# qimingfan10/Prov-gigapath-replication

Measured on AMD Instinct MI355X. Metric: slide-encoder tiles/sec at 1/2/4/8 GPUs (12L768d LongNet); attn MFMA util %, higher is better.
Workload: dtype bf16; 1 GPU; C3: gigapath_slide_enc12l768d forward, one 70000-tile slide per GPU, all_layer_embed=True; slides_per_gpu=1, parallelism=replica x1

## Files before the change

### include/gigapath_hip.h

```cpp
#ifndef GIGAPATH_HIP_H
#define GIGAPATH_HIP_H

#include <stddef.h>
#include <stdint.h>

#ifdef __cplusplus
extern "C" {
#endif

#define GP_ABI_VERSION 10
#define GP_EARG (-1)
#define GP_MAX_BRANCHES 8
#define GP_MAX_DESTS 8

#define GP_FMT_BF16 0
#define GP_FMT_F16 1
#define GP_FMT_F16_VBF16 2

int gp_abi_version(void);

const char* gp_last_error_string(void);

int gp_coords_to_pos(const void* coords, int coords_is_f64, int64_t n_tiles, int grid,
                     double tile_size, int64_t* pos, int32_t* err_count, void* stream);

// ... 63 lines not shown
int gp_branch_merge_ln_window(const uint16_t* const* o_in, const float* const* lse_in,
                              const int32_t* seg_len, const int32_t* ratios, int nbranch, int64_t B,
                              int64_t L, int64_t tok_lo, int64_t n_tok, int H, int D, const float* ln_w,
                              const float* ln_b, float eps, uint16_t* out, int fmt, void* stream);

int64_t gp_varlen_plan_bytes(int nslide, int nbranch);
int gp_varlen_plan(const int64_t* L, int nslide, int H, int D, const int32_t* seg_len,
                   const int32_t* ratios, int nbranch, const uint16_t* qkv, int64_t qkv_row_stride,
                   uint16_t* const* o_out, float* const* lse_out, void* plan_host, int64_t plan_bytes,
                   int64_t* o_elems, int64_t* lse_elems);
int gp_dilated_attn_fwd_varlen(const void* plan_host, const void* plan_dev, int q_log2_prescaled,
                               int fmt, void* stream);
int gp_branch_merge_ln_varlen(const void* plan_host, const void* plan_dev, const float* ln_w,
                              const float* ln_b, float eps, uint16_t* out, int fmt, void* stream);

int gp_residual_layernorm(float* x, const uint16_t* y, const float* bias, const float* ln_w,
                          const float* ln_b, float eps, uint16_t* ln_out, int64_t rows, int cols,
                          int fmt, void* stream);

int gp_residual2_layernorm(float* x, const uint16_t* y1, const float* b1, const uint16_t* y2, const float* b2,
                           const float* ln_w, const float* ln_b, float eps, uint16_t* ln_out, int64_t rows,
                           int cols, int fmt, void* stream);

int gp_gelu_layernorm(const uint16_t* h, const float* ln_w, const float* ln_b, float eps,
                      uint16_t* out, int64_t rows, int cols, int fmt, void* stream);

int64_t gp_gemm_workspace_bytes(int64_t M, int64_t N, int64_t K);

int gp_linear(const uint16_t* A, int64_t lda, const uint16_t* W, int64_t ldw, const float* bias,
              uint16_t* C, int64_t ldc, int64_t M, int64_t N, int64_t K, void* ws, int64_t ws_bytes,
// ... 43 lines not shown
```

### prov-gigapath-replication_amd/gigapath/_hip.py

```python
from __future__ import annotations

import ctypes
import os
from typing import Optional, Sequence

import torch

_HERE = os.path.dirname(os.path.abspath(__file__))
LIB_PATH = os.path.join(_HERE, "_lib", "libgigapath_hip.so")
ABI_VERSION = 10
MAX_BRANCHES = 8
MAX_DESTS = 8

c_i32, c_i64, c_f32, c_f64, c_vp = ctypes.c_int32, ctypes.c_int64, ctypes.c_float, ctypes.c_double, ctypes.c_void_p


class GpRowDest(ctypes.Structure):
    _fields_ = [("tok_lo", c_i64), ("tok_hi", c_i64), ("dst", c_vp)]


class GpAttnBranch(ctypes.Structure):
    _fields_ = [("seg_len", c_i32), ("ratio", c_i32), ("k", c_vp), ("v", c_vp), ("kv_row_stride", c_i64),
                ("kv_tok_base", c_i64), ("kv_sparse_cols", c_i32), ("o", c_vp), ("lse", c_vp),
                ("key_part", c_i32), ("key_parts", c_i32)]

# ... 7 lines not shown
    "gp_dilated_attn_fwd": [c_vp, c_vp, c_vp, c_i64, c_i64, c_i64, c_i32, c_i32, c_vp, c_vp, c_i32, c_vp, c_vp,
                            c_f32, c_i32, c_i32, c_vp],
    "gp_dilated_attn_fwd_ex": [c_vp, c_i64, c_i64, c_i64, c_i64, c_i32, c_i32, c_i64, c_i64, c_vp, c_i32, c_f32,
                               c_i32, c_i32, c_vp],
    "gp_attn_launch_params": [c_vp, c_i32],
    "gp_dilated_sparsify": [c_vp, c_i64, c_i64, c_i64, c_i64, c_i64, c_i64, c_i32, c_i32, c_vp, c_vp, c_i32, c_vp,
                            c_vp, c_vp],
    "gp_dilated_sparsify_dests": [c_vp, c_i64, c_i64, c_i64, c_i64, c_i64, c_i64, c_i32, c_i32, c_vp, c_vp, c_i32,
                                  c_vp, c_vp, c_vp],
    "gp_branch_merge_ln_window": [c_vp, c_vp, c_vp, c_vp, c_i32, c_i64, c_i64, c_i64, c_i64, c_i32, c_i32, c_vp, c_vp,
                                  c_f32, c_vp, c_i32, c_vp],
    "gp_seg_attn_fwd": [c_vp, c_vp, c_vp, c_i64, c_i64, c_i32, c_i32, c_f32, c_vp, c_vp, c_vp],
    "gp_seg_attn_fwd_f16": [c_vp, c_vp, c_vp, c_i64, c_i64, c_i32, c_i32, c_f32, c_vp, c_vp, c_vp],
    "gp_branch_merge_ln": [c_vp, c_vp, c_vp, c_vp, c_i32, c_i64, c_i64, c_i32, c_i32, c_vp, c_vp, c_f32, c_vp, c_i32,
                           c_vp],
    "gp_residual_layernorm": [c_vp, c_vp, c_vp, c_vp, c_vp, c_f32, c_vp, c_i64, c_i32, c_i32, c_vp],
    "gp_residual2_layernorm": [c_vp, c_vp, c_vp, c_vp, c_vp, c_vp, c_vp, c_f32, c_vp, c_i64, c_i32, c_i32, c_vp],
    "gp_gelu_layernorm": [c_vp, c_vp, c_vp, c_f32, c_vp, c_i64, c_i32, c_i32, c_vp],
    "gp_layernorm_f32": [c_vp, c_i64, c_vp, c_vp, c_f32, c_vp, c_i64, c_i32, c_vp],
    "gp_mean_tokens": [c_vp, c_i64, c_i64, c_i32, c_i64, c_vp, c_vp],
    "gp_varlen_plan_bytes": [c_i32, c_i32],
    "gp_varlen_plan": [c_vp, c_i32, c_i32, c_i32, c_vp, c_vp, c_i32, c_vp, c_i64, c_vp, c_vp, c_vp, c_i64, c_vp, c_vp],
    "gp_dilated_attn_fwd_varlen": [c_vp, c_vp, c_i32, c_i32, c_vp],
    "gp_branch_merge_ln_varlen": [c_vp, c_vp, c_vp, c_vp, c_f32, c_vp, c_i32, c_vp],
    "gp_gemm_workspace_bytes": [c_i64, c_i64, c_i64],
    "gp_linear": [c_vp, c_i64, c_vp, c_i64, c_vp, c_vp, c_i64, c_i64, c_i64, c_i64, c_vp, c_i64, c_i32, c_vp],
    "gp_ffn_fc1_gelu": [c_vp, c_i64, c_vp, c_i64, c_vp, c_vp, c_i64, c_vp, c_i64, c_i64, c_i64, c_i32, c_vp],
    "gp_ffn_fc2_ln": [c_vp, c_i64, c_vp, c_i64, c_vp, c_vp, c_vp, c_f32, c_vp, c_i64, c_i64, c_i64, c_i64, c_vp, c_i64,
                      c_i32, c_vp],
    "gp_linear_resid": [c_vp, c_i64, c_vp, c_i64, c_vp, c_vp, c_i64, c_vp, c_vp, c_vp, c_i64, c_vp, c_f32, c_vp, c_i64,
                        c_i64, c_i64, c_vp, c_i64, c_i32, c_vp],
    "gp_linear_ln": [c_vp, c_i64, c_vp, c_i64, c_vp, c_i32, c_vp, c_vp, c_f32, c_vp, c_vp, c_vp, c_i64, c_i64, c_i64,
                     c_i64, c_vp, c_i64, c_i32, c_vp],
    "gp_ffn_fc1_gelu_ln": [c_vp, c_i64, c_vp, c_i64, c_vp, c_i32, c_vp, c_vp, c_f32, c_vp, c_vp, c_vp, c_i64, c_vp,
                           c_i64, c_i64, c_i64, c_i32, c_vp],
    "gp_ffn_fc2_ln_resid": [c_vp, c_i64, c_vp, c_i64, c_vp, c_vp, c_vp, c_f32, c_vp, c_i64, c_vp, c_vp, c_vp, c_i64,
                            c_vp, c_f32, c_vp, c_i64, c_i64, c_i64, c_vp, c_i64, c_i32, c_vp],
}
_RESTYPES = {"gp_last_error_string": ctypes.c_char_p, "gp_varlen_plan_bytes": c_i64, "gp_gemm_workspace_bytes": c_i64}

_lib = None


class HipLibraryError(RuntimeError):
    pass


def load_library(path: Optional[str] = None) -> ctypes.CDLL:
    global _lib
    if _lib is not None and path is None:
        return _lib
    p = path or LIB_PATH
    if not os.path.exists(p):
        raise HipLibraryError(
# ... 209 lines not shown
        (lib.gp_seg_attn_fwd, "gp_seg_attn_fwd")
    _check(fn(_ptr(q), _ptr(k), _ptr(v), nb, sl, H, D, float(softmax_scale), _ptr(o), _ptr(lse), _stream()), name)


def branch_merge_ln(outs, lses, segs, ratios, B, L, H, D, ln_w, ln_b, eps, out):
    lib = load_library()
    fmt = fmt_of(out.dtype)
    _dev(out, name="out")
    for o in outs:
        _dev(o, out.dtype, "o")
    _check(lib.gp_branch_merge_ln(_ptr_array(outs), _ptr_array(lses), _i32_array(segs), _i32_array(ratios),
                                  len(segs), B, L, H, D, _ptr(ln_w), _ptr(ln_b), eps, _ptr(out), fmt, _stream()),
           "gp_branch_merge_ln")


def residual_layernorm(x, y, bias, ln_w, ln_b, eps, ln_out, rows, cols):
    lib = load_library()
    fmt = fmt_of(y.dtype)
    _dev(x, torch.float32, "x"); _dev(y, name="y")
    if ln_out is not None:
        _dev(ln_out, y.dtype, "ln_out")
    _check(lib.gp_residual_layernorm(_ptr(x), _ptr(y), _ptr(bias), _ptr(ln_w), _ptr(ln_b), eps, _ptr(ln_out),
                                     rows, cols, fmt, _stream()), "gp_residual_layernorm")


def residual2_layernorm(x, y1, b1, y2, b2, ln_w, ln_b, eps, ln_out, rows, cols):
    lib = load_library()
    fmt = fmt_of(y1.dtype)
    _dev(x, torch.float32, "x"); _dev(y1, name="y1")
    if y2 is not None:
# ... 252 lines not shown
```

### prov-gigapath-replication_amd/gigapath/runtime.py

```python
from __future__ import annotations

import functools
import math
import os
import threading
from collections import OrderedDict
from dataclasses import dataclass, field
from typing import Dict, List, Optional, Sequence, Tuple

import numpy as np
import torch

from . import _hip

_TUNED = os.path.join(os.path.dirname(os.path.abspath(__file__)), "tuned", "tunableop_results.csv")
_tuned_loaded = False


def use_tuned_gemms(dev=None):
    global _tuned_loaded
    path = os.environ.get("GIGAPATH_TUNED_GEMMS_FILE", _TUNED)
    if _tuned_loaded or os.environ.get("GIGAPATH_NO_TUNED_GEMMS") == "1" or not os.path.exists(path):
        return
    if dev is None or torch.device(dev).type != "cuda":
# ... 325 lines not shown
    with TIMER.span("gemm_out"):
        _hip.linear_resid(ws.a, pa.w_o, pa.b_o, ws.x, ws.shift[0], pl.ln2_w, ws.y, ws.xstats, ws.gemm_ws,
                          eps_next=pl.ln2_eps if mp else None, s_out=ws.shift[1] if mp else None)
    with TIMER.span("gemm_fc1"):
        _hip.ffn_fc1_gelu_ln(ws.y, pl.w1, ws.xstats, E // 256, pl.c1, pl.d1, pl.ln2_eps, ws.shift[0], ws.shift[1],
                             ws.f, ws.fstats, merged=mp)
    with TIMER.span("gemm_fc2"):
        last = nxt is None
        _hip.ffn_fc2_ln_resid(ws.f, pl.w2g, ws.fstats, pl.c2, pl.d2, pl.fln_eps, ws.x, ws.shift[1],
                              None if last else nxt.ln1_w, ws.y, ws.xstats, ws.gemm_ws,
                              eps_next=None if (last or not mp) else nxt.ln1_eps,
                              s_out=None if (last or not mp) else ws.shift[0])


def ffn_forward(pl: "PackedLayer", a: torch.Tensor, f: torch.Tensor, y: torch.Tensor, fstats, gemm_ws,
                M: int, F: int) -> Optional[torch.Tensor]:
    if pl.ffn_fused and fstats is not None:
        with TIMER.span("gemm_fc1"):
            _hip.ffn_fc1_gelu(a, pl.w1, pl.b1_f32, f, fstats)
        with TIMER.span("gemm_fc2"):
            _hip.ffn_fc2_ln(f, pl.w2g, fstats, pl.c2, pl.d2, pl.fln_eps, y, gemm_ws)
        return None
    with TIMER.span("gemm_fc1"), blaslt_serialized():
        torch.addmm(pl.b1, a, pl.w1.t(), out=f)
    with TIMER.span("gelu_ln"):
        _hip.gelu_layernorm(f, pl.fln_w, pl.fln_b, pl.fln_eps, f, M, F)
    with TIMER.span("gemm_fc2"), blaslt_serialized():
        torch.mm(f, pl.w2.t(), out=y)
    return pl.b2


def ffn_buffers(dev, M: int, E: int, F: int):
    if not (ffn_fusable(E, F) or resid_fusable(E, F)):
        return None, gemm_workspace(dev, M, E, F)
    stats = torch.empty((F // 256 + 1) * M * 2, dtype=torch.float32, device=dev)
    return stats, gemm_workspace(dev, M, E, F)


def gemm_workspace(dev, M: int, E: int, F: int) -> torch.Tensor:
    nb = 0
    if torch.device(dev).type == "cuda":
        shapes = [(E, F)] + ([(3 * E, E), (E, E)] if OWN_GEMMS else [])
# ... 32 lines not shown
            raise RuntimeError("varlen packing needs the pre-scaled q of D = 48")
        with TIMER.span("attn"):
            _hip.dilated_attn_fwd_varlen(scratch.plan, True, v_bf16=v_bf16)
        with TIMER.span("merge"):
            _hip.branch_merge_ln_varlen(scratch.plan, pa.ln_w if inner_ln else None, pa.ln_b if inner_ln else None,
                                        pa.ln_eps, out)
        return
    with TIMER.span("attn"):
        _hip.dilated_attn_fwd(qkv, qkv[:, E:], qkv[:, 2 * E:], 3 * E, B, L, H, D, pa.segs, pa.ratios,
                              scratch.outs, scratch.lses, 0.0, pa.prescaled, v_bf16=v_bf16)
    with TIMER.span("merge"):
        _hip.branch_merge_ln(scratch.outs, scratch.lses, pa.segs, pa.ratios, B, L, H, D,
                             pa.ln_w if inner_ln else None, pa.ln_b if inner_ln else None, pa.ln_eps, out)


class Workspace:
    def __init__(self, dev, B: int, L: int, E: int, F: int, H: int, segs, ratios, act: torch.dtype = torch.bfloat16):
        M = B * L
        self.key = (str(dev), B, L, E, F, H, tuple(segs), tuple(ratios), act)
        self.x = torch.empty(M, E, dtype=torch.float32, device=dev)
        self.a = torch.empty(M, E, dtype=act, device=dev)
        self.qkv = torch.empty(M, 3 * E, dtype=act, device=dev)
        self.y = torch.empty(M, E, dtype=act, device=dev)
        self.y2 = torch.empty(M, E, dtype=act, device=dev)
        self.f = torch.empty(M, F, dtype=act, device=dev)
        self.fstats, self.gemm_ws = ffn_buffers(dev, M, E, F)
        self.xstats, self.shift = resid_buffers(dev, M, E)
        self.attn = AttentionScratch(dev, B, L, H, E // H, segs, ratios, act)


class PackedWorkspace(Workspace):
# ... 4 lines not shown
        T = sum(self.Ls)
        M = T
        self.key = (str(dev), tuple(self.Ls), E, F, H, tuple(segs), tuple(ratios), act)
        self.x = torch.empty(M, E, dtype=torch.float32, device=dev)
        self.a = torch.empty(M, E, dtype=act, device=dev)
        self.qkv = torch.empty(M, 3 * E, dtype=act, device=dev)
        self.y = torch.empty(M, E, dtype=act, device=dev)
        self.y2 = torch.empty(M, E, dtype=act, device=dev)
        self.f = torch.empty(M, F, dtype=act, device=dev)
        self.fstats, self.gemm_ws = ffn_buffers(dev, M, E, F)
        self.xstats, self.shift = resid_buffers(dev, M, E)
        self.attn = VarlenScratch(dev, self.Ls, H, E // H, segs, ratios, self.qkv)
        self.tok_off = self.attn.plan.tok_off
        self.cls_idx = torch.tensor(self.tok_off[:-1], dtype=torch.int64, device=dev)


class EncoderEngine:

    def __init__(self):
        self._sig = None
        self.layers: List[PackedLayer] = []
        self._packs: Dict[torch.dtype, tuple] = {}
        self._ws: "OrderedDict[int, Workspace]" = OrderedDict()
        self._pws: "OrderedDict[int, PackedWorkspace]" = OrderedDict()
        self.ws: Optional[Workspace] = None
        self.pws: Optional[PackedWorkspace] = None

    def pack(self, encoder, dev, act: Optional[torch.dtype] = None):
        use_tuned_gemms(dev)
        act = act or act_dtype()
# ... 40 lines not shown
        return self.pws

    def stream_workspace(self, stream, packed: bool = False):
        table = self._pws if packed else self._ws
        return table.get(int(stream.cuda_stream)) if stream is not None else None

    def detach_workspace(self, ws) -> None:
        for table in (self._ws, self._pws):
            for k in [k for k, v in table.items() if v is ws]:
                table.pop(k)
        if self.ws is ws:
            self.ws = None
        if self.pws is ws:
            self.pws = None

    def run_layers(self, ws: Workspace, B: int, L: int, layer_hook=None, shift_ready: bool = False):
        M = B * L
        E = ws.x.shape[1]
        F = ws.f.shape[1]
        nl = len(self.layers)
        if self.layers and all(pl.resid_fused for pl in self.layers) and ws.fstats is not None:
            if not shift_ready:
                torch.mean(ws.x, 1, out=ws.shift[0])
            for li, pl in enumerate(self.layers):
                pa = pl.attn
                with TIMER.span("gemm_qkv"):
                    if li == 0:
                        linear(ws.a, pa.w_qkv, pa.b_qkv, pa.b_qkv_f32, ws.qkv, ws.gemm_ws, v_bf16=pa.v_bf16)
                    else:
                        fused_qkv(pl, ws, ws.qkv)
                dilated_attention_core(pa, ws.qkv, B, L, ws.attn, ws.a, v_bf16=pa.v_bf16)
                fused_post_attention(pl, self.layers[li + 1] if li + 1 < nl else None, ws)
                if layer_hook is not None:
                    layer_hook(li + 1)
            return
        for li, pl in enumerate(self.layers):
            pa = pl.attn
            with TIMER.span("gemm_qkv"):
                linear(ws.a, pa.w_qkv, pa.b_qkv, pa.b_qkv_f32, ws.qkv, ws.gemm_ws, v_bf16=pa.v_bf16)
            dilated_attention_core(pa, ws.qkv, B, L, ws.attn, ws.a, v_bf16=pa.v_bf16)
            with TIMER.span("gemm_out"):
                linear(ws.a, pa.w_o, None, None, ws.y, ws.gemm_ws)
            nxt = self.layers[li + 1] if li + 1 < nl else None
            residual_pair(pl, nxt, ws, M, E, F)
            if layer_hook is not None:
                layer_hook(li + 1)


RESID2 = os.environ.get("GIGAPATH_RESID2", "1") != "0"


def residual_pair(pl: "PackedLayer", nxt: Optional["PackedLayer"], ws, M: int, E: int, F: int):
    pa = pl.attn
    ln1 = (nxt.ln1_w, nxt.ln1_b, nxt.ln1_eps) if nxt else (None, None, 1e-5)
    if RESID2:
        with TIMER.span("resid_ln"):
            _hip.residual2_layernorm(ws.x, ws.y, pa.b_o, None, None, pl.ln2_w, pl.ln2_b, pl.ln2_eps, ws.a, M, E)
        b2 = ffn_forward(pl, ws.a, ws.f, ws.y2, ws.fstats, ws.gemm_ws, M, F)
        with TIMER.span("resid_ln"):
            _hip.residual2_layernorm(ws.x, ws.y, pa.b_o, ws.y2, b2, ln1[0], ln1[1], ln1[2], ws.a, M, E)
        return
    with TIMER.span("resid_ln"):
        _hip.residual_layernorm(ws.x, ws.y, pa.b_o, pl.ln2_w, pl.ln2_b, pl.ln2_eps, ws.a, M, E)
    b2 = ffn_forward(pl, ws.a, ws.f, ws.y, ws.fstats, ws.gemm_ws, M, F)
    with TIMER.span("resid_ln"):
        _hip.residual_layernorm(ws.x, ws.y, b2, ln1[0], ln1[1], ln1[2], ws.a, M, E)


def gemm_flops(B: int, N: int, E: int, F: int, C: int, depth: int) -> float:
    L = N + 1
    return float(2 * B * L * (4 * E * E + 2 * E * F) * depth + 2 * B * N * C * E)


def merge_bytes(L: int, segs: Sequence[int], ratios: Sequence[int], H: int, D: int, B: int = 1) -> float:
    E = H * D
    per_tok = sum(E / r * 2 + H / r * 4 for r in ratios) + E * 2
    return float(B * L * per_tok)


def attention_valid_flops_window(L: int, segs: Sequence[int], ratios: Sequence[int], H: int, D: int, lo: int,
                                 hi: int) -> float:
# ... 17 lines not shown
```

### prov-gigapath-replication_amd/gigapath/slide_encoder.py

```python
from __future__ import annotations

import os
from collections import OrderedDict
from functools import partial
from typing import Dict, List

import numpy as np
import torch
import torch.nn as nn

from . import _hip, runtime
from .pos_embed import axis_table, get_2d_sincos_pos_embed
from .torchscale.model.LongNet import make_longnet_from_name

_REGISTRY: Dict[str, callable] = {}


def register_model(fn):
    _REGISTRY[fn.__name__] = fn
    return fn


def list_models() -> List[str]:
    return sorted(_REGISTRY)
# ... 180 lines not shown
    def graph_stream(self):
        dev = self.cls_token.device
        key = (str(dev), int(torch.cuda.current_stream(dev).cuda_stream))
        if key not in self._capture_streams:
            while len(self._capture_streams) >= self.max_capture_streams:
                self._capture_streams.pop(next(iter(self._capture_streams)))
            self._capture_streams[key] = torch.cuda.Stream(device=dev)
        self._capture_streams.move_to_end(key)
        return self._capture_streams[key]

    def graph_entry(self, x, c, all_layer_embed):
        dev = self.cls_token.device
        self._packed_top(dev)
        self.encoder.engine.pack(self.encoder, dev)
        key = (str(dev), int(torch.cuda.current_stream(dev).cuda_stream), tuple(x.shape), x.dtype, c.dtype,
               runtime.act_dtype(), bool(all_layer_embed), bool(self.global_pool), self._top_sig,
               self.encoder.engine._sig)
        ent = self._graph_lookup(key)
        if ent is None and self._graph_wanted(key):
            ent = self._capture(key, x, c, lambda sx, sc: self._forward_device(sx, sc, all_layer_embed, False),
                                lambda st: self.encoder.engine.stream_workspace(st, packed=False))
        return ent

    def _graph_lookup(self, key):
        ent = self._graphs.get(key)
        if ent is not None:
            self._graphs.move_to_end(key)
        return ent

    def _graph_wanted(self, key) -> bool:
        if len(self._graph_seen) > 4096:
            self._graph_seen.clear()
# ... 91 lines not shown
        if self._sp is not None and self._sp.world > 1:
            raise ValueError("forward_packed is single-device: disable sequence parallelism first")
        if self.encoder.layers[0].self_attn.head_dim != 48 or len({c.dtype for c in cs}) != 1 or \
                len({x.dtype for x in xs}) != 1:
            return [self.forward(x[None], c[None], all_layer_embed) for x, c in zip(xs, cs)]
        Ns = tuple(int(x.shape[0]) for x in xs)
        x_cat = torch.cat(xs, 0)
        c_cat = torch.cat(cs, 0)
        if self.validate_positions:
            self.check_positions([c_cat])
        if self.use_hip_graphs and not runtime.TIMER.enabled:
            self._packed_top(dev)
            self.encoder.engine.pack(self.encoder, dev)
            key = ("packed", str(dev), int(torch.cuda.current_stream(dev).cuda_stream), Ns, x_cat.dtype,
                   c_cat.dtype, runtime.act_dtype(), bool(all_layer_embed), bool(self.global_pool),
                   self._top_sig, self.encoder.engine._sig)
            ent = self._graph_lookup(key)
            if ent is None and self._graph_wanted(key):
                ent = self._capture(key, x_cat, c_cat,
                                    lambda sx, sc: self._forward_packed_device(sx, sc, Ns, all_layer_embed),
                                    lambda st: self.encoder.engine.stream_workspace(st, packed=True))
            if ent is None:
                res = self._forward_packed_device(x_cat, c_cat, Ns, all_layer_embed)
            else:
                graph, sx, sc, res = ent
                sx.copy_(x_cat)
                sc.copy_(c_cat)
                runtime.replay_graph(graph)
                res = res.clone()
        else:
            res = self._forward_packed_device(x_cat, c_cat, Ns, all_layer_embed)
# ... 14 lines not shown
            ws.pos = torch.empty(Nt, dtype=torch.int64, device=dev)
        xp = ws.y[:Nt]
        self._patch_gemm(top, x_cat, xp, ws.gemm_ws)
        _hip.coords_to_pos(c_cat.contiguous(), self.slide_ngrids, self.tile_size, ws.pos, None)
        with runtime.TIMER.span("posembed"):
            n0 = 0
            for i, n in enumerate(Ns):
                t0 = ws.tok_off[i]
                _hip.posembed_cls_ln(xp[n0:n0 + n], ws.pos[n0:n0 + n], top["tab"], top["cls"], 1, n, E,
                                     self.slide_ngrids, top["ln1_w"], top["ln1_b"], top["ln1_eps"],
                                     ws.x[t0:t0 + n + 1], ws.a[t0:t0 + n + 1], ws.shift[0, t0:t0 + n + 1])
                n0 += n
        n_out = (1 + len(layers)) if all_layer_embed else 1
        res = torch.empty(n_out, S, E, dtype=torch.float32, device=dev)
        pool = torch.empty(S, E, dtype=torch.float32, device=dev)

        def readout(slot: int):
            if self.global_pool:
                for i, L in enumerate(Ls):
                    t0 = ws.tok_off[i]
                    _hip.mean_tokens(ws.x[t0:t0 + L], 1, L, E, 1, pool[i:i + 1])
            else:
                torch.index_select(ws.x, 0, ws.cls_idx, out=pool)
            _hip.layernorm_f32(pool, E, top["norm_w"], top["norm_b"], top["norm_eps"], res[slot], S, E)

        if all_layer_embed:
            readout(0)
        eng.run_layers(ws, 1, T, readout if all_layer_embed else None, shift_ready=True)
        if not all_layer_embed:
            if self.global_pool:
                _hip.layernorm_f32(ws.x, E, top["enc_w"], top["enc_b"], top["enc_eps"], ws.x, T, E)
                readout(0)
            else:
                cls_rows = torch.index_select(ws.x, 0, ws.cls_idx)
                _hip.layernorm_f32(cls_rows, E, top["enc_w"], top["enc_b"], top["enc_eps"], cls_rows, S, E)
                _hip.layernorm_f32(cls_rows, E, top["norm_w"], top["norm_b"], top["norm_eps"], res[0], S, E)
        return res

    def _forward_device(self, x, coords, all_layer_embed, validate):
        dev = self.cls_token.device
        B, N, C = x.shape
        E, L, M = self.embed_dim, N + 1, B * (N + 1)
        top = self._packed_top(dev)
        eng = self.encoder.engine
        layers = eng.pack(self.encoder, dev)
        pa = layers[0].attn
        ws = eng.workspace(dev, B, L, E, self.encoder.args.encoder_ffn_embed_dim, pa.H, pa.segs, pa.ratios)
        if not hasattr(ws, "pos") or ws.pos.numel() != B * N:
            ws.pos = torch.empty(B * N, dtype=torch.int64, device=dev)
# ... 2 lines not shown
        xp = ws.y[:B * N]
        self._patch_gemm(top, x.reshape(B * N, C), xp, ws.gemm_ws)
        c = coords if coords.dtype in (torch.float32, torch.float64) else coords.float()
        ws.err.zero_()
        _hip.coords_to_pos(c.contiguous(), self.slide_ngrids, self.tile_size, ws.pos, ws.err)
        if validate and int(ws.err.item()) > 0:
            raise IndexError("coords map outside pos_embed (%d rows): %d tiles" %
                             (self.slide_ngrids ** 2 + 1, int(ws.err.item())))
        with runtime.TIMER.span("posembed"):
            _hip.posembed_cls_ln(xp, ws.pos, top["tab"], top["cls"], B, N, E, self.slide_ngrids, top["ln1_w"],
                                 top["ln1_b"], top["ln1_eps"], ws.x, ws.a, ws.shift[0])

        n_out = (1 + len(layers)) if all_layer_embed else 1
        res = torch.empty(n_out, B, E, dtype=torch.float32, device=dev)
        pool = torch.empty(B, E, dtype=torch.float32, device=dev) if self.global_pool else None

        def readout(slot: int):
            if self.global_pool:
                _hip.mean_tokens(ws.x, B, L, E, 1, pool)
                _hip.layernorm_f32(pool, E, top["norm_w"], top["norm_b"], top["norm_eps"], res[slot], B, E)
            else:
                _hip.layernorm_f32(ws.x, L * E, top["norm_w"], top["norm_b"], top["norm_eps"], res[slot], B, E)

        if all_layer_embed:
            readout(0)
        eng.run_layers(ws, B, L, readout if all_layer_embed else None, shift_ready=True)
        if not all_layer_embed:
            if self.global_pool:
                _hip.layernorm_f32(ws.x, E, top["enc_w"], top["enc_b"], top["enc_eps"], ws.x, M, E)
                readout(0)
            else:
                cls_rows = torch.empty(B, E, dtype=torch.float32, device=dev)
                _hip.layernorm_f32(ws.x, L * E, top["enc_w"], top["enc_b"], top["enc_eps"], cls_rows, B, E)
                _hip.layernorm_f32(cls_rows, E, top["norm_w"], top["norm_b"], top["norm_eps"], res[0], B, E)
        out_dtype = self.norm.weight.dtype
        return [res[i].to(out_dtype) for i in range(n_out)]


    def _forward_sp(self, x, coords, all_layer_embed):
        sp = self._sp
        B, N, C = x.shape
        if B != 1:
            raise ValueError("sequence parallel forward takes one slide (B = 1), got B = %d" % B)
        dev = self.cls_token.device
        E, L = self.embed_dim, N + 1
        top = self._packed_top(dev)
        eng = self.encoder.engine
        layers = eng.pack(self.encoder, dev)
# ... 103 lines not shown
```

Before: 2.353 million tiles/s.

## Compute only CLS rows in the final encoder layer

In the last encoder layer, attention, out-projection, residual/LN and FFN are computed only for each slide's CLS token, since only CLS rows feed the readout when global_pool is off. A new HIP kernel pair does chunked split-softmax attention for the CLS query over each dilated branch's keys, then merges the branches with LayerNorm. This removes the full-sequence attention, GEMMs and FFN for the last of twelve layers over 70k tokens. It relies on no other consumer of the final layer's non-CLS token states, and it can be disabled with an environment variable.

```diff
diff --git a/include/gigapath_hip.h b/include/gigapath_hip.h
--- a/include/gigapath_hip.h
+++ b/include/gigapath_hip.h
@@ -8,7 +8,7 @@
 extern "C" {
 #endif
 
-#define GP_ABI_VERSION 10
+#define GP_ABI_VERSION 11
 #define GP_EARG (-1)
 #define GP_MAX_BRANCHES 8
 #define GP_MAX_DESTS 8
@@ -102,6 +102,14 @@
 int gp_branch_merge_ln_varlen(const void* plan_host, const void* plan_dev, const float* ln_w,
                               const float* ln_b, float eps, uint16_t* out, int fmt, void* stream);
 
+int64_t gp_cls_attn_workspace_bytes(int64_t max_len, int64_t nslide, int H, int D, const int32_t* seg_len,
+                                    const int32_t* ratios, int nbranch);
+int gp_cls_attn_merge_ln(const uint16_t* q, const uint16_t* k, const uint16_t* v, int64_t row_stride,
+                         const int64_t* slide_off, const int64_t* slide_len, int64_t nslide, int64_t max_len,
+                         int H, int D, const int32_t* seg_len, const int32_t* ratios, int nbranch,
+                         float softmax_scale, int q_log2_prescaled, int fmt, const float* ln_w,
+                         const float* ln_b, float eps, uint16_t* out, void* ws, int64_t ws_bytes, void* stream);
+
 int gp_residual_layernorm(float* x, const uint16_t* y, const float* bias, const float* ln_w,
                           const float* ln_b, float eps, uint16_t* ln_out, int64_t rows, int cols,
                           int fmt, void* stream);
diff --git a/prov-gigapath-replication_amd/csrc/gp_cls_attn.hip b/prov-gigapath-replication_amd/csrc/gp_cls_attn.hip
--- /dev/null
+++ b/prov-gigapath-replication_amd/csrc/gp_cls_attn.hip
@@ -0,0 +1,324 @@
+#include <math.h>
+
+#include <algorithm>
+
+#include "gp_api.h"
+#include "gp_common.h"
+
+namespace {
+
+constexpr int kChunk = 256;
+constexpr int kRecHead = 4;
+
+struct ClsArgs {
+  const uint16_t* q;
+  const uint16_t* k;
+  const uint16_t* v;
+  int64_t row_stride;
+  const int64_t* slide_off;
+  const int64_t* slide_len;
+  int64_t max_len;
+  int32_t H, D, nbranch, items;
+  int32_t sl[GP_MAX_BRANCHES];
+  int32_t r[GP_MAX_BRANCHES];
+  int32_t hpg[GP_MAX_BRANCHES];
+  int32_t mc[GP_MAX_BRANCHES];
+  int32_t pre[GP_MAX_BRANCHES + 1];
+  float qk_scale;
+  const float* ln_w;
+  const float* ln_b;
+  float eps;
+  uint16_t* out;
+  float* ws;
+};
+
+GP_DEV int cls_keys(const ClsArgs& a, int b, int64_t L) {
+  const int64_t s = a.sl[b] < L ? (int64_t)a.sl[b] : L;
+  return (int)((s + a.r[b] - 1) / a.r[b]);
+}
+GP_DEV int64_t cls_len(const ClsArgs& a, int slide) {
+  const int64_t L = a.slide_len[slide];
+  return L < 1 ? 1 : (L > a.max_len ? a.max_len : L);
+}
+
+template <bool kH16>
+GP_DEV void unpack8(const uint4 u, float* out) {
+  const uint32_t w[4] = {u.x, u.y, u.z, u.w};
+#pragma unroll
+  for (int j = 0; j < 4; ++j) {
+    out[2 * j] = e2f<kH16>(w[j] & 0xffffu);
+    out[2 * j + 1] = e2f_hi<kH16>(w[j]);
+  }
+}
+
+template <int D, bool kQK, bool kV>
+__global__ __launch_bounds__(kChunk) void cls_attn_partial_kernel(const ClsArgs a) {
+  __shared__ float red[4][D + 2];
+  const int slide = blockIdx.y;
+  int item = blockIdx.x, b = 0;
+  while (b + 1 < a.nbranch && item >= a.pre[b + 1]) ++b;
+  item -= a.pre[b];
+  const int h = item / a.mc[b];
+  const int c = item - h * a.mc[b];
+  const int64_t L = cls_len(a, slide);
+  const int m = cls_keys(a, b, L);
+  const int k0 = c * kChunk;
+  if (k0 >= m) return;
+  const int tid = threadIdx.x, lane = tid & 63, wv = tid >> 6;
+  const bool valid = k0 + tid < m;
+  const int64_t tok0 = a.slide_off[slide];
+  const int64_t tok = tok0 + (valid ? (int64_t)(k0 + tid) * a.r[b] : 0);
+  const uint4* kp = reinterpret_cast<const uint4*>(a.k + tok * a.row_stride + h * D);
+  const uint4* vp = reinterpret_cast<const uint4*>(a.v + tok * a.row_stride + h * D);
+  const uint4* qp = reinterpret_cast<const uint4*>(a.q + tok0 * a.row_stride + h * D);
+  uint4 kr[D / 8], vr[D / 8];
+#pragma unroll
+  for (int i = 0; i < D / 8; ++i) kr[i] = kp[i];
+#pragma unroll
+  for (int i = 0; i < D / 8; ++i) vr[i] = vp[i];
+  float dot = 0.f;
+#pragma unroll
+  for (int i = 0; i < D / 8; ++i) {
+    float qf[8], kf[8];
+    unpack8<kQK>(qp[i], qf);
+    unpack8<kQK>(kr[i], kf);
+#pragma unroll
+    for (int j = 0; j < 8; ++j) dot = __builtin_fmaf(qf[j], kf[j], dot);
+  }
+  const float s2 = valid ? dot * a.qk_scale : -INFINITY;
+  float mx = wave_max(s2);
+  if (lane == 0) red[wv][0] = mx;
+  __syncthreads();
+  mx = fmaxf(fmaxf(red[0][0], red[1][0]), fmaxf(red[2][0], red[3][0]));
+  const float p = valid ? exp2f(s2 - mx) : 0.f;
+  const float ps = wave_sum(p);
+#pragma unroll
+  for (int i = 0; i < D / 8; ++i) {
+    float vf[8];
+    unpack8<kV>(vr[i], vf);
+#pragma unroll
+    for (int j = 0; j < 8; ++j) {
+      const float t = wave_sum(valid ? p * vf[j] : 0.f);
+      if (lane == 0) red[wv][2 + 8 * i + j] = t;
+    }
+  }
+  if (lane == 0) red[wv][1] = ps;
+  __syncthreads();
+  float* rec = a.ws + ((int64_t)slide * a.items + blockIdx.x) * (D + kRecHead);
+  if (tid < D) rec[kRecHead + tid] = (red[0][2 + tid] + red[1][2 + tid]) + (red[2][2 + tid] + red[3][2 + tid]);
+  if (tid == D) rec[0] = mx;
+  if (tid == D + 1) rec[1] = (red[0][1] + red[1][1]) + (red[2][1] + red[3][1]);
+}
+
+constexpr int kMergeWaves = 16;
+
+GP_DEV float block_sum(float v, float* red, int tid) {
+  v = wave_sum(v);
+  __syncthreads();
+  if ((tid & 63) == 0) red[tid >> 6] = v;
+  __syncthreads();
+  float t = 0.f;
+#pragma unroll
+  for (int w = 0; w < kMergeWaves; ++w) t += red[w];
+  return t;
+}
+
+template <bool kH>
+__global__ __launch_bounds__(64 * kMergeWaves) void cls_merge_ln_kernel(const ClsArgs a) {
+  extern __shared__ float smem[];
+  const int H = a.H, D = a.D, E = H * D, nbr = a.nbranch;
+  float* o_s = smem;
+  float* lse_s = smem + nbr * E;
+  float* red = lse_s + nbr * H;
+  const int slide = blockIdx.x;
+  const int tid = threadIdx.x, lane = tid & 63, wv = tid >> 6;
+  const int64_t L = cls_len(a, slide);
+  const int rs = D + kRecHead;
+  int pair = 0;
+  for (int b = 0; b < nbr; ++b) {
+    const int nch = (cls_keys(a, b, L) + kChunk - 1) / kChunk;
+    for (int h = 0; h < a.hpg[b]; ++h, ++pair) {
+      if (pair % kMergeWaves != wv) continue;
+      const float* rec = a.ws + ((int64_t)slide * a.items + a.pre[b] + h * a.mc[b]) * rs;
+      float mx = -INFINITY;
+      for (int c = lane; c < nch; c += 64) mx = fmaxf(mx, rec[c * rs]);
+      mx = wave_max(mx);
+      float sum = 0.f, acc0 = 0.f, acc1 = 0.f;
+      for (int c0 = 0; c0 < nch; c0 += 64) {
+        const int c = c0 + lane;
+        const float f = c < nch ? exp2f(rec[c * rs] - mx) : 0.f;
+        if (c < nch) sum = __builtin_fmaf(rec[c * rs + 1], f, sum);
+        const int n = nch - c0 < 64 ? nch - c0 : 64;
+        for (int cc = 0; cc < n; cc += 8) {
+          float x0[8], x1[8], fc[8];
+#pragma unroll
+          for (int j = 0; j < 8; ++j) {
+            const int ci = cc + j < n ? cc + j : n - 1;
+            const float* r = rec + (c0 + ci) * rs + kRecHead;
+            x0[j] = lane < D ? r[lane] : 0.f;
+            x1[j] = lane + 64 < D ? r[lane + 64] : 0.f;
+            const float fj = __shfl(f, ci, 64);
+            fc[j] = cc + j < n ? fj : 0.f;
+          }
+#pragma unroll
+          for (int j = 0; j < 8; ++j) {
+            acc0 = __builtin_fmaf(x0[j], fc[j], acc0);
+            acc1 = __builtin_fmaf(x1[j], fc[j], acc1);
+          }
+        }
+      }
+      sum = wave_sum(sum);
+      if (lane < D) o_s[(b * H + h) * D + lane] = e2f<kH>(f2e<kH>(acc0 / sum));
+      if (lane + 64 < D) o_s[(b * H + h) * D + lane + 64] = e2f<kH>(f2e<kH>(acc1 / sum));
+      if (lane == 0) lse_s[b * H + h] = (mx + log2f(sum)) * 0.69314718055994530942f;
+    }
+  }
+  __syncthreads();
+  constexpr int kMaxPairs = 1;
+  constexpr int kStep = 128 * kMergeWaves;
+  float val[kMaxPairs][2];
+  float part = 0.f;
+#pragma unroll
+  for (int i = 0; i < kMaxPairs; ++i) {
+    const int e = 2 * tid + i * kStep;
+    val[i][0] = val[i][1] = 0.f;
+    if (e < E) {
+      const int h = e / D;
+      float lse[GP_MAX_BRANCHES];
+      float mx = -INFINITY;
+#pragma unroll
+      for (int b = 0; b < GP_MAX_BRANCHES; ++b) {
+        float l = (b < nbr && h < a.hpg[b]) ? lse_s[b * H + h] : -1e8f;
+        if (l == 0.f) l = -1e8f;
+        lse[b] = l;
+        if (b < nbr) mx = fmaxf(mx, l);
+      }
+      float wsum = 0.f;
+#pragma unroll
+      for (int b = 0; b < GP_MAX_BRANCHES; ++b)
+        if (b < nbr) {
+          lse[b] = expf(lse[b] - mx);
+          wsum += lse[b];
+        }
+#pragma unroll
+      for (int b = 0; b < GP_MAX_BRANCHES; ++b)
+        if (b < nbr && h < a.hpg[b]) {
+          const float w = lse[b] / wsum;
+          val[i][0] = __builtin_fmaf(o_s[b * E + e], w, val[i][0]);
+          val[i][1] = __builtin_fmaf(o_s[b * E + e + 1], w, val[i][1]);
+        }
+      part += val[i][0] + val[i][1];
+    }
+  }
+  if (a.ln_w != nullptr) {
+    const float mean = block_sum(part, red, tid) / (float)E;
+    float q = 0.f;
+#pragma unroll
+    for (int i = 0; i < kMaxPairs; ++i)
+      if (2 * tid + i * kStep < E) {
+        const float d0 = val[i][0] - mean, d1 = val[i][1] - mean;
+        q += d0 * d0 + d1 * d1;
+      }
+    const float rstd = rsqrtf(block_sum(q, red, tid) / (float)E + a.eps);
+#pragma unroll
+    for (int i = 0; i < kMaxPairs; ++i) {
+      const int e = 2 * tid + i * kStep;
+      if (e < E) {
+        val[i][0] = (val[i][0] - mean) * rstd * a.ln_w[e] + a.ln_b[e];
+        val[i][1] = (val[i][1] - mean) * rstd * a.ln_w[e + 1] + a.ln_b[e + 1];
+      }
+    }
+  }
+#pragma unroll
+  for (int i = 0; i < kMaxPairs; ++i) {
+    const int e = 2 * tid + i * kStep;
+    if (e < E)
+      *reinterpret_cast<uint32_t*>(a.out + (int64_t)slide * E + e) = pack2e<kH>(val[i][0], val[i][1]);
+  }
+}
+
+int64_t cls_plan(ClsArgs& a, int64_t max_len, int H, const int32_t* seg_len, const int32_t* ratios, int nbranch) {
+  int64_t items = 0;
+  for (int b = 0; b < nbranch; ++b) {
+    if (seg_len[b] < 1 || ratios[b] < 1) return -1;
+    const GpBranch g = gp_make_branch(max_len, seg_len[b], ratios[b], H);
+    a.sl[b] = seg_len[b];
+    a.r[b] = ratios[b];
+    a.hpg[b] = std::min(g.hpg, H);
+    a.mc[b] = (g.m + kChunk - 1) / kChunk;
+    a.pre[b] = (int32_t)items;
+    items += (int64_t)a.hpg[b] * a.mc[b];
+    if (items > 0x3fffffff) return -1;
+  }
+  a.pre[nbranch] = (int32_t)items;
+  a.items = (int32_t)items;
+  return items;
+}
+
+bool cls_shape_ok(int64_t max_len, int64_t nslide, int H, int D, int nbranch) {
+  return max_len >= 1 && nslide >= 1 && nslide <= 65535 && H >= 1 && (D == 48 || D == 64 || D == 96) &&
+         (int64_t)H * D <= 1536 && nbranch >= 1 && nbranch <= GP_MAX_BRANCHES;
+}
+
+template <int D>
+void launch_partial(const ClsArgs& a, int fmt, dim3 grid, hipStream_t s) {
+  if (fmt == GP_FMT_BF16) cls_attn_partial_kernel<D, false, false><<<grid, kChunk, 0, s>>>(a);
+  else if (fmt == GP_FMT_F16) cls_attn_partial_kernel<D, true, true><<<grid, kChunk, 0, s>>>(a);
+  else cls_attn_partial_kernel<D, true, false><<<grid, kChunk, 0, s>>>(a);
+}
+
+}
+
+extern "C" int64_t gp_cls_attn_workspace_bytes(int64_t max_len, int64_t nslide, int H, int D, const int32_t* seg_len,
+                                               const int32_t* ratios, int nbranch) {
+  if (!cls_shape_ok(max_len, nslide, H, D, nbranch) || !seg_len || !ratios) return -1;
+  ClsArgs a = {};
+  const int64_t items = cls_plan(a, max_len, H, seg_len, ratios, nbranch);
+  return items < 0 ? -1 : nslide * items * (D + kRecHead) * (int64_t)sizeof(float);
+}
+
+extern "C" int gp_cls_attn_merge_ln(const uint16_t* q, const uint16_t* k, const uint16_t* v, int64_t row_stride,
+                                    const int64_t* slide_off, const int64_t* slide_len, int64_t nslide,
+                                    int64_t max_len, int H, int D, const int32_t* seg_len, const int32_t* ratios,
+                                    int nbranch, float softmax_scale, int q_log2_prescaled, int fmt,
+                                    const float* ln_w, const float* ln_b, float eps, uint16_t* out, void* ws,
+                                    int64_t ws_bytes, void* stream) {
+  gp_clear_error();
+  GP_REQUIRE(fmt == GP_FMT_BF16 || fmt == GP_FMT_F16 || fmt == GP_FMT_F16_VBF16, "gp_cls_attn_merge_ln: bad fmt %d", fmt);
+  GP_REQUIRE(cls_shape_ok(max_len, nslide, H, D, nbranch),
+             "gp_cls_attn_merge_ln: bad shape (max_len %lld, nslide %lld, H %d, D %d in {48, 64, 96}, H*D <= 1536, "
+             "nbranch %d)", (long long)max_len, (long long)nslide, H, D, nbranch);
+  GP_REQUIRE(q && k && v && slide_off && slide_len && seg_len && ratios && out && ws,
+             "gp_cls_attn_merge_ln: null pointer");
+  GP_REQUIRE((ln_w == nullptr) == (ln_b == nullptr), "gp_cls_attn_merge_ln: ln_w and ln_b go together");
+  GP_REQUIRE(row_stride >= (int64_t)H * D && row_stride % 8 == 0 && gp_aligned(q, 16) && gp_aligned(k, 16) &&
+                 gp_aligned(v, 16) && gp_aligned(out, 4) && gp_aligned(ws, 16),
+             "gp_cls_attn_merge_ln: q / k / v rows must be 16-byte aligned (row_stride %% 8 == 0)");
+  ClsArgs a = {};
+  const int64_t items = cls_plan(a, max_len, H, seg_len, ratios, nbranch);
+  GP_REQUIRE(items > 0, "gp_cls_attn_merge_ln: bad segment schedule");
+  const int64_t need = nslide * items * (D + kRecHead) * (int64_t)sizeof(float);
+  GP_REQUIRE(ws_bytes >= need, "gp_cls_attn_merge_ln: workspace of %lld bytes, %lld needed", (long long)ws_bytes,
+             (long long)need);
+  a.q = q; a.k = k; a.v = v;
+  a.row_stride = row_stride;
+  a.slide_off = slide_off;
+  a.slide_len = slide_len;
+  a.max_len = max_len;
+  a.H = H; a.D = D; a.nbranch = nbranch;
+  a.qk_scale = q_log2_prescaled ? 1.0f
+                                : (softmax_scale > 0.f ? softmax_scale : 1.0f / sqrtf((float)D)) * 1.4426950408889634f;
+  a.ln_w = ln_w; a.ln_b = ln_b; a.eps = eps;
+  a.out = out;
+  a.ws = static_cast<float*>(ws);
+  hipStream_t s = gp_stream(stream);
+  const dim3 grid((unsigned)items, (unsigned)nslide);
+  if (D == 48) launch_partial<48>(a, fmt, grid, s);
+  else if (D == 64) launch_partial<64>(a, fmt, grid, s);
+  else launch_partial<96>(a, fmt, grid, s);
+  if (int rc = gp_check_launch("gp_cls_attn_merge_ln (partial)")) return rc;
+  const size_t lds = ((size_t)nbranch * H * D + (size_t)nbranch * H + kMergeWaves) * sizeof(float);
+  if (fmt == GP_FMT_BF16) cls_merge_ln_kernel<false><<<(unsigned)nslide, 64 * kMergeWaves, lds, s>>>(a);
+  else cls_merge_ln_kernel<true><<<(unsigned)nslide, 64 * kMergeWaves, lds, s>>>(a);
+  return gp_check_launch("gp_cls_attn_merge_ln (merge)");
+}
diff --git a/prov-gigapath-replication_amd/gigapath/_hip.py b/prov-gigapath-replication_amd/gigapath/_hip.py
--- a/prov-gigapath-replication_amd/gigapath/_hip.py
+++ b/prov-gigapath-replication_amd/gigapath/_hip.py
@@ -8,7 +8,7 @@
 
 _HERE = os.path.dirname(os.path.abspath(__file__))
 LIB_PATH = os.path.join(_HERE, "_lib", "libgigapath_hip.so")
-ABI_VERSION = 10
+ABI_VERSION = 11
 MAX_BRANCHES = 8
 MAX_DESTS = 8
 
@@ -46,6 +46,9 @@
     "gp_seg_attn_fwd_f16": [c_vp, c_vp, c_vp, c_i64, c_i64, c_i32, c_i32, c_f32, c_vp, c_vp, c_vp],
     "gp_branch_merge_ln": [c_vp, c_vp, c_vp, c_vp, c_i32, c_i64, c_i64, c_i32, c_i32, c_vp, c_vp, c_f32, c_vp, c_i32,
                            c_vp],
+    "gp_cls_attn_workspace_bytes": [c_i64, c_i64, c_i32, c_i32, c_vp, c_vp, c_i32],
+    "gp_cls_attn_merge_ln": [c_vp, c_vp, c_vp, c_i64, c_vp, c_vp, c_i64, c_i64, c_i32, c_i32, c_vp, c_vp, c_i32, c_f32,
+                             c_i32, c_i32, c_vp, c_vp, c_f32, c_vp, c_vp, c_i64, c_vp],
     "gp_residual_layernorm": [c_vp, c_vp, c_vp, c_vp, c_vp, c_f32, c_vp, c_i64, c_i32, c_i32, c_vp],
     "gp_residual2_layernorm": [c_vp, c_vp, c_vp, c_vp, c_vp, c_vp, c_vp, c_f32, c_vp, c_i64, c_i32, c_i32, c_vp],
     "gp_gelu_layernorm": [c_vp, c_vp, c_vp, c_f32, c_vp, c_i64, c_i32, c_i32, c_vp],
@@ -69,7 +72,8 @@
     "gp_ffn_fc2_ln_resid": [c_vp, c_i64, c_vp, c_i64, c_vp, c_vp, c_vp, c_f32, c_vp, c_i64, c_vp, c_vp, c_vp, c_i64,
                             c_vp, c_f32, c_vp, c_i64, c_i64, c_i64, c_vp, c_i64, c_i32, c_vp],
 }
-_RESTYPES = {"gp_last_error_string": ctypes.c_char_p, "gp_varlen_plan_bytes": c_i64, "gp_gemm_workspace_bytes": c_i64}
+_RESTYPES = {"gp_last_error_string": ctypes.c_char_p, "gp_varlen_plan_bytes": c_i64, "gp_gemm_workspace_bytes": c_i64,
+             "gp_cls_attn_workspace_bytes": c_i64}
 
 _lib = None
 
@@ -309,6 +313,33 @@
            "gp_branch_merge_ln")
 
 
+def cls_attn_workspace_bytes(max_len, nslide, H, D, segs, ratios) -> int:
+    nb = int(load_library().gp_cls_attn_workspace_bytes(int(max_len), int(nslide), H, D, _i32_array(segs),
+                                                        _i32_array(ratios), len(segs)))
+    if nb < 0:
+        raise ValueError("cls_attn_workspace_bytes: bad shape (max_len %d, nslide %d, H %d, D %d, %d branches)"
+                         % (max_len, nslide, H, D, len(segs)))
+    return nb
+
+
+def cls_attn_merge_ln(q, k, v, row_stride, slide_off, slide_len, max_len, H, D, segs, ratios, ln_w, ln_b, eps, out,
+                      ws, softmax_scale=0.0, q_log2_prescaled=False, v_bf16=False):
+    lib = load_library()
+    fmt = qkv_fmt_of(q.dtype, v_bf16)
+    for t in (q, k, v):
+        if not t.is_cuda or t.dtype != q.dtype:
+            raise TypeError("q/k/v must be device tensors of one 16-bit dtype")
+    _dev(slide_off, torch.int64, "slide_off"); _dev(slide_len, torch.int64, "slide_len")
+    n = slide_off.numel()
+    if slide_len.numel() != n or out.numel() != n * H * D:
+        raise ValueError("cls_attn_merge_ln: slide_off, slide_len and out [nslide, H*D] disagree on nslide")
+    _dev(out, q.dtype, "out"); _dev(ws, torch.uint8, "ws")
+    _check(lib.gp_cls_attn_merge_ln(_ptr(q), _ptr(k), _ptr(v), row_stride, _ptr(slide_off), _ptr(slide_len), n,
+                                    int(max_len), H, D, _i32_array(segs), _i32_array(ratios), len(segs),
+                                    float(softmax_scale), int(bool(q_log2_prescaled)), fmt, _ptr(ln_w), _ptr(ln_b),
+                                    eps, _ptr(out), _ptr(ws), ws.numel(), _stream()), "gp_cls_attn_merge_ln")
+
+
 def residual_layernorm(x, y, bias, ln_w, ln_b, eps, ln_out, rows, cols):
     lib = load_library()
     fmt = fmt_of(y.dtype)
diff --git a/prov-gigapath-replication_amd/gigapath/runtime.py b/prov-gigapath-replication_amd/gigapath/runtime.py
--- a/prov-gigapath-replication_amd/gigapath/runtime.py
+++ b/prov-gigapath-replication_amd/gigapath/runtime.py
@@ -1,5 +1,6 @@
 from __future__ import annotations
 
+import contextlib
 import functools
 import math
 import os
@@ -363,18 +364,19 @@
 
 
 def ffn_forward(pl: "PackedLayer", a: torch.Tensor, f: torch.Tensor, y: torch.Tensor, fstats, gemm_ws,
-                M: int, F: int) -> Optional[torch.Tensor]:
+                M: int, F: int, timed: bool = True) -> Optional[torch.Tensor]:
+    span = TIMER.span if timed else (lambda name: contextlib.nullcontext())
     if pl.ffn_fused and fstats is not None:
-        with TIMER.span("gemm_fc1"):
+        with span("gemm_fc1"):
             _hip.ffn_fc1_gelu(a, pl.w1, pl.b1_f32, f, fstats)
-        with TIMER.span("gemm_fc2"):
+        with span("gemm_fc2"):
             _hip.ffn_fc2_ln(f, pl.w2g, fstats, pl.c2, pl.d2, pl.fln_eps, y, gemm_ws)
         return None
-    with TIMER.span("gemm_fc1"), blaslt_serialized():
+    with span("gemm_fc1"), blaslt_serialized():
         torch.addmm(pl.b1, a, pl.w1.t(), out=f)
-    with TIMER.span("gelu_ln"):
+    with span("gelu_ln"):
         _hip.gelu_layernorm(f, pl.fln_w, pl.fln_b, pl.fln_eps, f, M, F)
-    with TIMER.span("gemm_fc2"), blaslt_serialized():
+    with span("gemm_fc2"), blaslt_serialized():
         torch.mm(f, pl.w2.t(), out=y)
     return pl.b2
 
@@ -437,7 +439,40 @@
                              pa.ln_w if inner_ln else None, pa.ln_b if inner_ln else None, pa.ln_eps, out)
 
 
+class ClsRows:
+
+    def __init__(self, dev, offs: Sequence[int], lens: Sequence[int], E: int, F: int, H: int, segs, ratios,
+                 act: torch.dtype):
+        n = len(offs)
+        self.n, self.max_len = n, int(max(lens))
+        self.off = torch.tensor([int(o) for o in offs], dtype=torch.int64, device=dev)
+        self.len = torch.tensor([int(l) for l in lens], dtype=torch.int64, device=dev)
+        self.x = torch.empty(n, E, dtype=torch.float32, device=dev)
+        self.a = torch.empty(n, E, dtype=act, device=dev)
+        self.y = torch.empty(n, E, dtype=act, device=dev)
+        self.y2 = torch.empty(n, E, dtype=act, device=dev)
+        self.f = torch.empty(n, F, dtype=act, device=dev)
+        self.fstats, self.gemm_ws = ffn_buffers(dev, n, E, F)
+        self.attn_ws = torch.empty(_hip.cls_attn_workspace_bytes(self.max_len, n, H, E // H, segs, ratios),
+                                   dtype=torch.uint8, device=dev)
+
+
 class Workspace:
+    cls: Optional[ClsRows] = None
+
+    def cls_rows(self) -> ClsRows:
+        if self.cls is None:
+            dev, E, F = self.x.device, self.x.shape[1], self.f.shape[1]
+            segs, ratios, act = self.key[-3], self.key[-2], self.key[-1]
+            H = self.key[-4]
+            offs, lens = self._slides()
+            self.cls = ClsRows(dev, offs, lens, E, F, H, segs, ratios, act)
+        return self.cls
+
+    def _slides(self):
+        B, L = self.key[1], self.key[2]
+        return [b * L for b in range(B)], [L] * B
+
     def __init__(self, dev, B: int, L: int, E: int, F: int, H: int, segs, ratios, act: torch.dtype = torch.bfloat16):
         M = B * L
         self.key = (str(dev), B, L, E, F, H, tuple(segs), tuple(ratios), act)
@@ -472,6 +507,9 @@
         self.tok_off = self.attn.plan.tok_off
         self.cls_idx = torch.tensor(self.tok_off[:-1], dtype=torch.int64, device=dev)
 
+    def _slides(self):
+        return self.tok_off[:-1], self.Ls
+
 
 class EncoderEngine:
 
@@ -542,7 +580,8 @@
         if self.pws is ws:
             self.pws = None
 
-    def run_layers(self, ws: Workspace, B: int, L: int, layer_hook=None, shift_ready: bool = False):
+    def run_layers(self, ws: Workspace, B: int, L: int, layer_hook=None, shift_ready: bool = False,
+                   cls_rows: Optional[ClsRows] = None):
         M = B * L
         E = ws.x.shape[1]
         F = ws.f.shape[1]
@@ -557,8 +596,11 @@
                         linear(ws.a, pa.w_qkv, pa.b_qkv, pa.b_qkv_f32, ws.qkv, ws.gemm_ws, v_bf16=pa.v_bf16)
                     else:
                         fused_qkv(pl, ws, ws.qkv)
-                dilated_attention_core(pa, ws.qkv, B, L, ws.attn, ws.a, v_bf16=pa.v_bf16)
-                fused_post_attention(pl, self.layers[li + 1] if li + 1 < nl else None, ws)
+                if cls_rows is not None and li + 1 == nl:
+                    cls_tail(pl, ws, cls_rows)
+                else:
+                    dilated_attention_core(pa, ws.qkv, B, L, ws.attn, ws.a, v_bf16=pa.v_bf16)
+                    fused_post_attention(pl, self.layers[li + 1] if li + 1 < nl else None, ws)
                 if layer_hook is not None:
                     layer_hook(li + 1)
             return
@@ -566,6 +608,11 @@
             pa = pl.attn
             with TIMER.span("gemm_qkv"):
                 linear(ws.a, pa.w_qkv, pa.b_qkv, pa.b_qkv_f32, ws.qkv, ws.gemm_ws, v_bf16=pa.v_bf16)
+            if cls_rows is not None and li + 1 == nl:
+                cls_tail(pl, ws, cls_rows)
+                if layer_hook is not None:
+                    layer_hook(li + 1)
+                continue
             dilated_attention_core(pa, ws.qkv, B, L, ws.attn, ws.a, v_bf16=pa.v_bf16)
             with TIMER.span("gemm_out"):
                 linear(ws.a, pa.w_o, None, None, ws.y, ws.gemm_ws)
@@ -593,6 +640,24 @@
     b2 = ffn_forward(pl, ws.a, ws.f, ws.y, ws.fstats, ws.gemm_ws, M, F)
     with TIMER.span("resid_ln"):
         _hip.residual_layernorm(ws.x, ws.y, b2, ln1[0], ln1[1], ln1[2], ws.a, M, E)
+
+
+CLS_TAIL = os.environ.get("GIGAPATH_CLS_TAIL", "1") != "0"
+
+
+def cls_tail(pl: "PackedLayer", ws, c: ClsRows):
+    pa = pl.attn
+    n, E, F = c.n, pa.E, c.f.shape[1]
+    q, k, v = ws.qkv, ws.qkv[:, E:], ws.qkv[:, 2 * E:]
+    with TIMER.span("cls_attn"):
+        _hip.cls_attn_merge_ln(q, k, v, 3 * E, c.off, c.len, c.max_len, pa.H, pa.D, pa.segs, pa.ratios, pa.ln_w,
+                               pa.ln_b, pa.ln_eps, c.a, c.attn_ws, 0.0, pa.prescaled, v_bf16=pa.v_bf16)
+    with TIMER.span("cls_tail"):
+        torch.index_select(ws.x, 0, c.off, out=c.x)
+        linear(c.a, pa.w_o, None, None, c.y, c.gemm_ws)
+        _hip.residual2_layernorm(c.x, c.y, pa.b_o, None, None, pl.ln2_w, pl.ln2_b, pl.ln2_eps, c.a, n, E)
+        b2 = ffn_forward(pl, c.a, c.f, c.y2, c.fstats, c.gemm_ws, n, F, timed=False)
+        _hip.residual2_layernorm(c.x, c.y, pa.b_o, c.y2, b2, None, None, 1e-5, c.a, n, E)
 
 
 def gemm_flops(B: int, N: int, E: int, F: int, C: int, depth: int) -> float:
diff --git a/prov-gigapath-replication_amd/gigapath/slide_encoder.py b/prov-gigapath-replication_amd/gigapath/slide_encoder.py
--- a/prov-gigapath-replication_amd/gigapath/slide_encoder.py
+++ b/prov-gigapath-replication_amd/gigapath/slide_encoder.py
@@ -218,8 +218,8 @@
         self._packed_top(dev)
         self.encoder.engine.pack(self.encoder, dev)
         key = (str(dev), int(torch.cuda.current_stream(dev).cuda_stream), tuple(x.shape), x.dtype, c.dtype,
-               runtime.act_dtype(), bool(all_layer_embed), bool(self.global_pool), self._top_sig,
-               self.encoder.engine._sig)
+               runtime.act_dtype(), bool(all_layer_embed), bool(self.global_pool), bool(runtime.CLS_TAIL),
+               self._top_sig, self.encoder.engine._sig)
         ent = self._graph_lookup(key)
         if ent is None and self._graph_wanted(key):
             ent = self._capture(key, x, c, lambda sx, sc: self._forward_device(sx, sc, all_layer_embed, False),
@@ -341,7 +341,7 @@
             self.encoder.engine.pack(self.encoder, dev)
             key = ("packed", str(dev), int(torch.cuda.current_stream(dev).cuda_stream), Ns, x_cat.dtype,
                    c_cat.dtype, runtime.act_dtype(), bool(all_layer_embed), bool(self.global_pool),
-                   self._top_sig, self.encoder.engine._sig)
+                   bool(runtime.CLS_TAIL), self._top_sig, self.encoder.engine._sig)
             ent = self._graph_lookup(key)
             if ent is None and self._graph_wanted(key):
                 ent = self._capture(key, x_cat, c_cat,
@@ -386,25 +386,29 @@
         n_out = (1 + len(layers)) if all_layer_embed else 1
         res = torch.empty(n_out, S, E, dtype=torch.float32, device=dev)
         pool = torch.empty(S, E, dtype=torch.float32, device=dev)
+        cls = ws.cls_rows() if (runtime.CLS_TAIL and not self.global_pool) else None
 
         def readout(slot: int):
             if self.global_pool:
                 for i, L in enumerate(Ls):
                     t0 = ws.tok_off[i]
                     _hip.mean_tokens(ws.x[t0:t0 + L], 1, L, E, 1, pool[i:i + 1])
+            elif cls is not None and slot == len(layers):
+                _hip.layernorm_f32(cls.x, E, top["norm_w"], top["norm_b"], top["norm_eps"], res[slot], S, E)
+                return
             else:
                 torch.index_select(ws.x, 0, ws.cls_idx, out=pool)
             _hip.layernorm_f32(pool, E, top["norm_w"], top["norm_b"], top["norm_eps"], res[slot], S, E)
 
         if all_layer_embed:
             readout(0)
-        eng.run_layers(ws, 1, T, readout if all_layer_embed else None, shift_ready=True)
+        eng.run_layers(ws, 1, T, readout if all_layer_embed else None, shift_ready=True, cls_rows=cls)
         if not all_layer_embed:
             if self.global_pool:
                 _hip.layernorm_f32(ws.x, E, top["enc_w"], top["enc_b"], top["enc_eps"], ws.x, T, E)
                 readout(0)
             else:
-                cls_rows = torch.index_select(ws.x, 0, ws.cls_idx)
+                cls_rows = cls.x.clone() if cls is not None else torch.index_select(ws.x, 0, ws.cls_idx)
                 _hip.layernorm_f32(cls_rows, E, top["enc_w"], top["enc_b"], top["enc_eps"], cls_rows, S, E)
                 _hip.layernorm_f32(cls_rows, E, top["norm_w"], top["norm_b"], top["norm_eps"], res[0], S, E)
         return res
@@ -437,24 +441,28 @@
         n_out = (1 + len(layers)) if all_layer_embed else 1
         res = torch.empty(n_out, B, E, dtype=torch.float32, device=dev)
         pool = torch.empty(B, E, dtype=torch.float32, device=dev) if self.global_pool else None
+        cls = ws.cls_rows() if (runtime.CLS_TAIL and not self.global_pool) else None
 
         def readout(slot: int):
             if self.global_pool:
                 _hip.mean_tokens(ws.x, B, L, E, 1, pool)
                 _hip.layernorm_f32(pool, E, top["norm_w"], top["norm_b"], top["norm_eps"], res[slot], B, E)
+            elif cls is not None and slot == len(layers):
+                _hip.layernorm_f32(cls.x, E, top["norm_w"], top["norm_b"], top["norm_eps"], res[slot], B, E)
             else:
                 _hip.layernorm_f32(ws.x, L * E, top["norm_w"], top["norm_b"], top["norm_eps"], res[slot], B, E)
 
         if all_layer_embed:
             readout(0)
-        eng.run_layers(ws, B, L, readout if all_layer_embed else None, shift_ready=True)
+        eng.run_layers(ws, B, L, readout if all_layer_embed else None, shift_ready=True, cls_rows=cls)
         if not all_layer_embed:
             if self.global_pool:
                 _hip.layernorm_f32(ws.x, E, top["enc_w"], top["enc_b"], top["enc_eps"], ws.x, M, E)
                 readout(0)
             else:
                 cls_rows = torch.empty(B, E, dtype=torch.float32, device=dev)
-                _hip.layernorm_f32(ws.x, L * E, top["enc_w"], top["enc_b"], top["enc_eps"], cls_rows, B, E)
+                src, stride = (cls.x, E) if cls is not None else (ws.x, L * E)
+                _hip.layernorm_f32(src, stride, top["enc_w"], top["enc_b"], top["enc_eps"], cls_rows, B, E)
                 _hip.layernorm_f32(cls_rows, E, top["norm_w"], top["norm_b"], top["norm_eps"], res[0], B, E)
         out_dtype = self.norm.weight.dtype
         return [res[i].to(out_dtype) for i in range(n_out)]
```

Result: faster. 2.526 million tiles/s (median of 6 runs) (+7.3%).
